# NLESC-JCER/Fortran_Davidson

Hardware: AMD Instinct MI355X
Metric: Davidson iterations/sec (dense DPR solve, matrix resident in HBM) + A*V HBM GB/s vs roofline (higher is better)
Workload: dtype f64

## Files before the change

### fortran_davidson_amd/csrc/engine_apply.hip

```cpp
#include "engine_internal.h"

bool inner_f32_tiles(E* e, OpDesc& o) {
  if (e->inner_bits != 32 || o.kind != DAV_KIND_DENSE || o.storage != 1 || o.a32_refused) return false;
  if (o.a32_valid) return true;
  const size_t count = (size_t)std::max<int64_t>(e->sym.ntiles, 1) * SYM_TB * SYM_TB;
  if (!o.a32 && pool_malloc(&o.a32, sizeof(float) * count) != hipSuccess) {
    (void)hipGetLastError();
    o.a32 = nullptr;
    o.a32_refused = true;
    return false;
  }
  launch_tiles_to_f32(e->stream, o.a, o.a32, (int64_t)count);
  o.a32_valid = true;
  return true;
}

static double* sym_slab_t(const E* e, const SymLaunch& L) { return e->sym_slab + (int64_t)L.ngroups * L.dstride; }
static void sym_sweep(E* e, const SymLaunch& L, const OpDesc& o, const SymSet& set, const double* xt) {
  if (L.nitems == 0) return;
  const SymPlan* pl = L.plan;
  const void* tiles = L.use32 ? (const void*)o.a32 : (const void*)o.a;
  double *slabD = e->sym_slab, *slabT = sym_slab_t(e, L);
  const int64_t xs = e->xt_group_stride, ds = L.dstride, ts = L.tstride;
  switch (L.family) {
    case SYM_ROW_STORED:
      return launch_matvec_sym(e->stream, o.a, set.row_off, set.items, set.nitems, xt, L.kk, slabD, slabT, L.ngroups, xs, ds, ts);
    case SYM_ROW_GENERATED:
      return launch_matvec_sym_generated(e->stream, op_params(o), e->n, set.items, set.nitems, xt, L.kk, slabD, slabT, L.ngroups, xs, ds, ts);
    case SYM_SUPER:
      return launch_matvec_sym9(e->stream, L.R, o.kind != DAV_KIND_DENSE, tiles, L.use32, set.row_off, o.kind != DAV_KIND_DENSE ? op_params(o) : OpParams{},
                                e->n, e->sym_nb, pl->items, pl->nitems, pl->zslot_begin, xt, L.kk, slabD, slabT, L.nwg, xs, ds, ts, e->tune.sym_mfma4 != 0);
    case SYM_WIDE:
    case SYM_WIDE_F32:
      return launch_matvec_symw(e->stream, L.nbw, L.tall, L.use32, tiles, set.row_off, e->sym_nb, pl->items, pl->nitems, pl->zslot_begin, xt, L.kk, slabD, slabT, L.nwg, xs, ds, ts);
    case SYM_WIDE_GENERATED:
      return launch_matvec_symw_generated(e->stream, op_params(o), e->n, e->sym_nb, pl->items, pl->nitems, pl->zslot_begin, xt, L.kk, slabD, slabT, L.nwg, xs, ds, ts);
  }
}

static void count_apply(E* e, int which, int kk) { if (which == DAV_OP_A) { e->st.applies += 1; e->st.apply_cols += kk; } }

static int pack_operand(E* e, const double* src, int kk, bool gather) {
  launch_pack_xt(e->stream, src, e->ldp, e->nloc, e->nslab, kk, e->xt, e->xt_group_stride, e->row0);
  if (!gather) return 0;
  const int ngroups = (kk + 15) / 16;
  CollGroup grp(e);
  CHK(grp.begin(5, 8.0 * (double)e->nslab * 16 * ngroups * e->nranks));
  for (int g = 0; g < ngroups; ++g)
    CHK(coll_allgather(e, e->xt + g * e->xt_group_stride + e->row0 * 16, e->xt + g * e->xt_group_stride, (size_t)e->nslab * 16));
  return grp.end("all-gather of the new block", e->stream);
}

static void sym_reduce_groups(E* e, const SymLaunch& L, const SymSet& set, const int64_t* owned, double* out, int64_t chunk_rows, bool accumulate) {
  const int64_t total_rows = (int64_t)e->nranks * e->nslab;
  const double* slabT = sym_slab_t(e, L);
  for (int g = 0; g < L.ngroups; ++g) {
    const int kg = std::min(16, L.kk - 16 * g);
    const double *d = e->sym_slab + g * L.dstride, *t = slabT + g * L.tstride;
    double* og = out + (size_t)g * 16 * (size_t)(chunk_rows ? total_rows : e->ldp);
    if (L.plan)
      launch_sym9_reduce(e->stream, d, t, L.plan->row_begin, L.plan->zslot_begin, owned, L.plan->next_owned, L.R, e->sym_nb, e->nloc, kg, og, e->ldp,
                         chunk_rows, total_rows, accumulate);
    else
      launch_sym_reduce(e->stream, d, t, set.row_begin, owned, e->sym_nb, e->nloc, kg, og, e->ldp, chunk_rows, total_rows, accumulate);
  }
}

static int ensure_sym_wpart(E* e) {
  if (e->sym_wpart) return 0;
  HIPCHK(pool_malloc(&e->sym_wpart, sizeof(double) * (size_t)e->nranks * (size_t)e->nslab * 64));
  HIPCHK(pool_malloc(&e->sym_wrecv, sizeof(double) * (size_t)e->nslab * 64));
  return 0;
}

static int sym_scatter_to_panel(E* e, int kk, double* dst, bool accumulate, const char* what, double* h0 = nullptr, size_t h0_count = 0) {
  const size_t wstride = (size_t)e->nranks * (size_t)e->nslab * 16, rstride = (size_t)e->nslab * 16;
  const int ngroups = (kk + 15) / 16;
  CollGroup grp(e);
  CHK(grp.begin(6, 8.0 * (double)e->nslab * kk * e->nranks));
  for (int g = 0; g < ngroups; ++g)
    CHK(coll_reduce_scatter(e, e->sym_wpart + g * wstride, e->sym_wrecv + g * rstride, (size_t)e->nslab * std::min(16, kk - 16 * g)));
  if (h0) CHK(coll_allreduce(e, h0, h0_count));
  CHK(grp.end(what, e->stream));
  for (int g = 0; g < ngroups; ++g)
    launch_chunk_to_panel(e->stream, e->sym_wrecv + g * rstride, e->nslab, e->nloc, e->nloc_pad, std::min(16, kk - 16 * g), dst + (int64_t)(16 * g) * e->ldp, e->ldp, accumulate);
  return 0;
}

static double sym_stored_bytes(const E* e, const OpDesc& o, const SymSet& set, bool partial, bool use32) {
  return o.kind != DAV_KIND_DENSE ? 0.0 : (use32 ? 4.0 : 8.0) * (partial ? (double)set.ntiles * SYM_TB * SYM_TB : 0.5 * (double)e->n * ((double)e->n + 1.0) / e->nranks);
}

static int apply_sym_overlapped(E* e, int which, OpDesc& o, const double* src, int k, double* dst, bool timed, bool inner) {
  const int step = 32;
  const int nchunks = (k + step - 1) / step;
// ... 535 lines not shown
```

### fortran_davidson_amd/csrc/engine_comm.hip

```cpp
#include "engine_internal.h"

Rccl g_rccl;
int rccl_load() {
  if (g_rccl.lib) return 0;
  void* lib = dlopen("librccl.so", RTLD_NOW | RTLD_LOCAL);
  if (!lib) lib = dlopen("/opt/rocm/lib/librccl.so", RTLD_NOW | RTLD_LOCAL);
  if (!lib) return fail(std::string("cannot load librccl.so: ") + dlerror());
#define SYM(field, name)                                              \
  *(void**)(&g_rccl.field) = dlsym(lib, name);                        \
  if (!g_rccl.field) return fail(std::string("librccl.so lacks ") + name);
  SYM(GetUniqueId, "ncclGetUniqueId")
  SYM(CommInitRank, "ncclCommInitRank")
  SYM(CommDestroy, "ncclCommDestroy")
  SYM(AllGather, "ncclAllGather")
  SYM(AllReduce, "ncclAllReduce")
  SYM(Broadcast, "ncclBroadcast")
  SYM(ReduceScatter, "ncclReduceScatter")
  SYM(Send, "ncclSend")
  SYM(Recv, "ncclRecv")
  SYM(GroupStart, "ncclGroupStart")
  SYM(GroupEnd, "ncclGroupEnd")
  SYM(GetErrorString, "ncclGetErrorString")
  SYM(CommCount, "ncclCommCount")
#undef SYM
// ... 99 lines not shown
};
static void lg_release_turn(LocalGroup* g, int rank) {
  if (!g->serialize || g->segment[rank] == 0) return;
  const uint64_t pos = (uint64_t)((rank - g->first + g->n) % g->n);
  { std::lock_guard<std::mutex> lk(g->mu); g->turn = std::max(g->turn, g->segment[rank] * (uint64_t)g->n + pos + 1); }
  g->cv.notify_all();
}
static void lg_acquire_turn(LocalGroup* g, int rank) {
  if (!g->serialize) return;
  g->segment[rank] += 1;
  const uint64_t pos = (uint64_t)((rank - g->first + g->n) % g->n);
  const uint64_t ticket = g->segment[rank] * (uint64_t)g->n + pos;
  std::unique_lock<std::mutex> lk(g->mu);
  if (pos == 0 && g->turn < ticket) g->turn = ticket;
  g->cv.notify_all();
  g->cv.wait(lk, [&] { return g->turn >= ticket; });
}

struct ShmHeader {
  pthread_barrier_t bar;
  int nranks;
  size_t slot_doubles;
};
struct ShmGroup {
  ShmHeader* hdr = nullptr;
  double* slots = nullptr;
  size_t bytes = 0;
  std::string name;
  bool owner = false;
};

bool has_test_transport(const E* e) { return e->lg != nullptr || e->shm != nullptr; }
size_t test_transport_max_message(const E* e) { return e->shm ? e->shm->hdr->slot_doubles : (size_t)-1; }

int test_allgather(E* e, const double* send, double* recv, size_t count) {
  if (e->lg) {
    LocalGroup* g = e->lg;
    HIPCHK(hipStreamSynchronize(e->stream));
    lg_release_turn(g, e->rank);
    g->send[e->rank] = send;
    pthread_barrier_wait(&g->bar);
    for (int p = 0; p < g->n; ++p)
      if (recv + (size_t)p * count != g->send[p])
        HIPCHK(hipMemcpyAsync(recv + (size_t)p * count, g->send[p], sizeof(double) * count, hipMemcpyDeviceToDevice, e->stream));
    HIPCHK(hipStreamSynchronize(e->stream));
    pthread_barrier_wait(&g->bar);
    lg_acquire_turn(g, e->rank);
    return 0;
  }
  if (e->shm) {
    ShmGroup* g = e->shm;
    if (count > g->hdr->slot_doubles) return fail("shared-memory transport: message larger than a slot");
    HIPCHK(hipMemcpyAsync(g->slots + (size_t)e->rank * g->hdr->slot_doubles, send, sizeof(double) * count, hipMemcpyDeviceToHost, e->stream));
    HIPCHK(hipStreamSynchronize(e->stream));
    pthread_barrier_wait(&g->hdr->bar);
    for (int p = 0; p < e->nranks; ++p)
      if (p != e->rank || recv + (size_t)p * count != send)
        HIPCHK(hipMemcpyAsync(recv + (size_t)p * count, g->slots + (size_t)p * g->hdr->slot_doubles, sizeof(double) * count,
                              hipMemcpyHostToDevice, e->stream));
    HIPCHK(hipStreamSynchronize(e->stream));
    pthread_barrier_wait(&g->hdr->bar);
    return 0;
  }
  return fail("no test transport");
}

// ... 124 lines not shown
    for (int tries = 0; tries < 3000 && __atomic_load_n(&g->hdr->nranks, __ATOMIC_ACQUIRE) != e->nranks; ++tries) usleep(10000);
    if (__atomic_load_n(&g->hdr->nranks, __ATOMIC_ACQUIRE) != e->nranks) { munmap(p, bytes); delete g; return fail("dav_comm_init_shm: rank 0 did not initialise the segment"); }
  }
  e->shm = g;
  pthread_barrier_wait(&g->hdr->bar);
  return 0;
}

extern "C" int dav_local_group_yield(dav_handle_t e) {
  if (!e || !e->lg) return 0;
  (void)hipSetDevice(e->device);
  (void)hipStreamSynchronize(e->stream);
  lg_release_turn(e->lg, e->rank);
  return 0;
}

extern "C" int dav_local_group_join(dav_handle_t* handles, int n) {
  if (!handles || n < 1 || n > 16) return fail("dav_local_group_join: 1..16 engines");
  for (int r = 0; r < n; ++r)
    if (!handles[r] || handles[r]->nranks != n || handles[r]->rank != r || handles[r]->lg || handles[r]->comm)
      return fail("dav_local_group_join: engine r must be created with rank r of n and have no transport yet");
  LocalGroup* g = new LocalGroup();
  g->n = n;
  if (const char* ev = getenv("DAV_TEST_SERIALIZE")) g->serialize = ev[0] == '1';
  if (const char* ev = getenv("DAV_TEST_SERIALIZE_FIRST")) g->first = std::max(0, std::min(n - 1, atoi(ev)));
  pthread_barrier_init(&g->bar, nullptr, (unsigned)n);
  for (int r = 0; r < n; ++r) handles[r]->lg = g;
  return 0;
}

#else
bool has_test_transport(const E*) { return false; }
size_t test_transport_max_message(const E*) { return (size_t)-1; }
int test_allgather(E*, const double*, double*, size_t) { return fail("built without test transports"); }
int test_allreduce(E*, double*, size_t) { return fail("built without test transports"); }
int test_reduce_scatter(E*, const double*, double*, size_t) { return fail("built without test transports"); }
void shm_release(E*) {}
#endif

#if DAV_TEST_TRANSPORTS
__global__ void watchdog_stall_kernel(unsigned long long ticks) {
  const unsigned long long t0 = __builtin_amdgcn_s_memrealtime();
  while (__builtin_amdgcn_s_memrealtime() - t0 < ticks) __builtin_amdgcn_s_sleep(64);
}
#endif
int watch_mark(E* e, const char* what, hipStream_t stream) {
  Watchdog* w = e->wd;
  if (!w || e->group_depth > 0) return 0;
#if DAV_TEST_TRANSPORTS
  static const long stall_ms = [] { const char* ev = getenv("DAV_TEST_STALL_MS"); return ev ? atol(ev) : 0L; }();
  static const long stall_from = [] { const char* ev = getenv("DAV_TEST_STALL_FROM"); return ev ? atol(ev) : 0L; }();
  if (stall_ms > 0 && (long)w->seq >= stall_from)
    hipLaunchKernelGGL(watchdog_stall_kernel, dim3(1), dim3(1), 0, stream, (unsigned long long)stall_ms * 100000ull);
#endif
  std::lock_guard<std::mutex> lk(w->mu);
  Watchdog::Lane* l = nullptr;
  for (Watchdog::Lane& c : w->lane)
    if (c.used && c.stream == stream) { l = &c; break; }
  if (!l)
    for (Watchdog::Lane& c : w->lane)
      if (!c.used) { c.used = true; c.stream = stream; l = &c; break; }
  if (!l) return fail("collective watchdog: more streams than lanes");
  Watchdog::Mark& m = l->check_active ? l->latest : l->check;
  HIPCHK(hipEventRecord(m.ev, stream));
  m.what = what; m.seq = w->seq++; m.t0 = wall_seconds(); m.iter = e->iter_hint;
  if (l->check_active) l->latest_valid = true;
// ... 144 lines not shown
```

### fortran_davidson_amd/csrc/engine_internal.h

```cpp
#pragma once
#include "davidson_hip_private.h"
#include "kernels.h"
#include "ingest.h"

#include <dlfcn.h>
#include <fcntl.h>
#include <pthread.h>
#include <sys/mman.h>
#include <sys/stat.h>
#include <unistd.h>
#include <rccl/rccl.h>

#include <algorithm>
#include <chrono>
#include <condition_variable>
#include <ctime>
#include <mutex>
#include <cmath>
#include <cstdio>
#include <cstring>
#include <numeric>
#include <string>
#include <thread>
#include <vector>
// ... 130 lines not shown
  int64_t res_tiles = 0;
  int res_first = 0;
  bool res_decided = false;
  bool pass_res = false, pass_gen = false;
  SymSet* res = nullptr;
  SymSet* gen = nullptr;
  dav_device_apply_fn dev_fn = nullptr;
  void* dev_ctx = nullptr;
  SparseStore sp;
};

struct SmallBuf {
  double* dev = nullptr;
  double* host = nullptr;
  hipEvent_t done = nullptr;
  bool pending = false;
};

constexpr int N_SMALL = 4;
constexpr int N_EVPAIRS = 64;

struct Tune {
  int sym_wide = 2;
  int sym_wide32 = 1;
  int sym_pair = 1;
  int sym_quad = 1;
  int sym_overlap = 0;
  int sym_r = 0;
  int sym_tall = 1;
  int sym_gen_wide = 1;
  int sym_run = 0;
  int sym_run9 = 0;
  int sym_mfma4 = 1;
  int64_t mv_target = 0;
  int64_t mv_nsplit = 0;
  int gram_wgs = 0;
  int pg_pin = 1;
  int coll_direct = 0;
  int b_resident = 1;
  bool gjd_trace = false;
  int coll_select = 1;
  int coll_trial_corrupt = 0;
  bool coll_forced = false;
  int no_h0 = 0;
  int harness_libm = 0;
  int cheb_fuse = 1;
};
Tune tune_from_env();

enum { COLL_PATH_UNDECIDED = -1, COLL_PATH_PROGRAM_ORDER = 0, COLL_PATH_DIRECT = 1, COLL_PATH_SECOND_STREAM = 2 };
struct CollTrial {
  bool ran = false;
  int selected = COLL_PATH_PROGRAM_ORDER, columns = 0;
  double ms[3] = {0, 0, 0}, ms_max[3] = {0, 0, 0};
  bool valid[3] = {true, false, false}, valid_all[3] = {true, false, false};
  double differing[3] = {0, 0, 0}, maxdiff[3] = {0, 0, 0};
  std::string message[3];
};

enum { GUESS_NONE = 0, GUESS_ONE_SHOT = 1, GUESS_RESULT = 2 };
struct Watchdog;
struct dav_engine {
  Tune tune;
  int device = 0;
  hipStream_t stream = nullptr;
  int64_t n = 0, nslab = 0, nloc = 0, row0 = 0, nloc_pad = 0, ncols_pad = 0;
// ... 99 lines not shown
  bool stop = false;
  uint64_t seq = 0;
  double timeout_s = 0.0;
  int device = 0, rank = 0, nranks = 1;
};

static inline int method_kind(int code) { return code > 0 && (code & 0xff) == DAV_METHOD_CHEB ? DAV_METHOD_CHEB : code; }
static inline int64_t roundup(int64_t x, int64_t m) { return (x + m - 1) / m * m; }

struct SmallMat {
  const double* src; int64_t ld; int p, q;
  double* dev; int64_t ldm;
  bool image = false;
};

int bind(E* e);
int collect_events(E* e);
int timed_begin(E* e, int kind, double bytes, int* slot);
int timed_end(E* e, int slot);
int timed_begin_on(E* e, int kind, double bytes, int* slot, hipStream_t stream);
int timed_end_on(E* e, int slot, hipStream_t stream);
int small_upload(E* e, int i, const double* src, int64_t ld, int p, int q, int64_t* ldm_out);
int small_upload_multi(E* e, int i, SmallMat* mats, int n);
int small_upload_image(E* e, int i, const double* src, int64_t ld, int p, int q, int64_t* tp_out);
double* panel_ptr(E* e, int panel, int col);
int check_panel(E* e, int panel, int c0, int k);
int create_impl(E* e, int device, int64_t n, int max_cols, int gev, int rank, int nranks);
double wall_seconds();
void watchdog_loop(Watchdog* w);
bool has_comm(E* e);
int need_comm(E* e);
bool has_test_transport(const E* e);
size_t test_transport_max_message(const E* e);
int test_allgather(E* e, const double* send, double* recv, size_t count);
int test_allreduce(E* e, double* buf, size_t count);
int test_reduce_scatter(E* e, const double* send, double* recv, size_t count);
void shm_release(E* e);
int watch_mark(E* e, const char* what, hipStream_t stream);
int coll_group_begin(E* e);
int coll_group_end(E* e, const char* what, hipStream_t stream);
void coll_group_abort(E* e);
struct CollGroup {
  E* e; bool open = false; int slot = -1;
  explicit CollGroup(E* e_) : e(e_) {}
  int begin(int kind = 0, double bytes = 0.0, hipStream_t stream = nullptr) {
    if (kind != 0) {
      int rc = timed_begin_on(e, kind, bytes, &slot, stream ? stream : e->stream);
      if (rc != 0) return rc;
      e->st.collectives += 1;
      e->group_timed = true;
    }
    int rc = coll_group_begin(e); open = rc == 0; return rc;
  }
  int end(const char* what, hipStream_t stream) {
    open = false;
    e->group_timed = false;
    int rc = coll_group_end(e, what, stream);
    if (rc != 0) return rc;
    return timed_end_on(e, slot, stream);
  }
  ~CollGroup() { e->group_timed = false; if (open) coll_group_abort(e); }
};
int coll_allgather(E* e, const double* send, double* recv, size_t count);
int coll_allreduce(E* e, double* buf, size_t count);
int coll_reduce_scatter(E* e, const double* send, double* recv, size_t count);
int refresh_diag_host(E* e, int which);
// ... 42 lines not shown
```

### fortran_davidson_amd/csrc/k_matvec_sym9.hip

```cpp
#include "kernels.h"
#include <cstdlib>
#include <type_traits>

__device__ __forceinline__ const double* sym9_tile(const double* tiles, const int64_t* __restrict__ row_off, int I, int J) {
  return tiles + (row_off[I] + J) * (int64_t)(SYM_TB * SYM_TB);
}

__device__ __forceinline__ double mfma4_f64(double a, double b, double c) { return __builtin_amdgcn_mfma_f64_4x4x4f64(a, b, c, 0, 0, 0); }

template <int R, bool GEN, bool F32, bool M4, int HARN = 0>
__global__ __launch_bounds__(512, 1) void matvec_sym9_kernel(const void* __restrict__ tiles_v, const int64_t* __restrict__ row_off,
                                                             const int* __restrict__ items,
                                                             const int* __restrict__ zslot_begin, const double* __restrict__ xt,
                                                             double* __restrict__ slabD, double* __restrict__ slabT, int kcols,
                                                             int npair, int64_t xt_gstride, int64_t slabD_gstride,
                                                             int64_t slabT_gstride, int nb, OpParams op, int64_t n) {
  const double* tiles = static_cast<const double*>(tiles_v);
  const float* tiles32 = static_cast<const float*>(tiles_v);
  (void)tiles; (void)tiles32;
  constexpr int NCG = 4 / R;
  constexpr int NRS = 2 * R;
  constexpr int BW = 16 * NCG;
  constexpr int UPJ = SYM_TB / BW;
  constexpr int UPS = 64 / BW;
// ... 324 lines not shown
                     kcols, npair, xt_gstride, slabD_gstride, slabT_gstride, nb, op, n)
  const bool harness = gen && op.kind == DAV_KIND_HARNESS;
  const bool hsin = harness && op.trig != 0;
  const bool hlibm = harness && op.libm != 0;
  if (R == 4) {
    if (hlibm) DAV_SYM9_LAUNCH(4, true, false, true, 3);
    else if (hsin) DAV_SYM9_LAUNCH(4, true, false, true, 2);
    else if (harness) DAV_SYM9_LAUNCH(4, true, false, true, 1);
    else if (gen) DAV_SYM9_LAUNCH(4, true, false, true);
    else if (tiles_f32) DAV_SYM9_LAUNCH(4, false, true, true);
    else if (m4) DAV_SYM9_LAUNCH(4, false, false, true);
    else DAV_SYM9_LAUNCH(4, false, false, false);
  } else {
    if (hlibm) DAV_SYM9_LAUNCH(2, true, false, false, 3);
    else if (hsin) DAV_SYM9_LAUNCH(2, true, false, false, 2);
    else if (harness) DAV_SYM9_LAUNCH(2, true, false, false, 1);
    else if (gen) DAV_SYM9_LAUNCH(2, true, false, false);
    else if (tiles_f32) DAV_SYM9_LAUNCH(2, false, true, false);
    else DAV_SYM9_LAUNCH(2, false, false, false);
  }
#undef DAV_SYM9_LAUNCH
}

__global__ __launch_bounds__(256) void tiles_to_f32_kernel(const double* __restrict__ src, float* __restrict__ dst, int64_t count4) {
  for (int64_t e = (int64_t)blockIdx.x * 256 + threadIdx.x; e < count4; e += (int64_t)gridDim.x * 256) {
    const f64x2 a = reinterpret_cast<const f64x2*>(src)[2 * e], b = reinterpret_cast<const f64x2*>(src)[2 * e + 1];
    reinterpret_cast<float4*>(dst)[e] = float4{(float)a.x, (float)a.y, (float)b.x, (float)b.y};
  }
}
void launch_tiles_to_f32(hipStream_t st, const double* src, float* dst, int64_t count) {
  hipLaunchKernelGGL(tiles_to_f32_kernel, dim3(256 * 32), dim3(256), 0, st, src, dst, count / 4);
}

__global__ __launch_bounds__(256) void sym9_reduce_kernel(const double* __restrict__ slabD, const double* __restrict__ slabT,
                                                          const int* __restrict__ row_item_begin, const int* __restrict__ zslot_begin,
                                                          const int64_t* __restrict__ owned, const int* __restrict__ next_owned, int R, int nb,
                                                          int nsuper, int64_t nloc, int k, double* __restrict__ dst, int64_t ldd,
                                                          int64_t chunk_rows, int64_t total_rows, int accumulate) {
  const int J = blockIdx.x, col = blockIdx.y, r = threadIdx.x;
  if (col >= k) return;
  double sum = 0.0;
  const int Sown = J / R, sub = J % R;
  for (int it = row_item_begin[Sown]; it < row_item_begin[Sown + 1]; ++it)
    sum += slabD[(((int64_t)it * R + sub) * 16 + col) * SYM_TB + r];
  auto zt = [&](int S) { return slabT[(((int64_t)zslot_begin[S] + J) * 16 + col) * SYM_TB + r]; };
  double s0 = 0.0, s1 = 0.0, s2 = 0.0, s3 = 0.0;
  const int Send = (nb - 1 > J) ? nsuper : 0;
  if (!owned) {
    int S = (J + 1) / R;
    for (; S + 3 < Send; S += 4) { s0 += zt(S); s1 += zt(S + 1); s2 += zt(S + 2); s3 += zt(S + 3); }
    for (; S < Send; ++S) s0 += zt(S);
  } else {
    int S = (J + 1) / R < nsuper ? next_owned[(J + 1) / R] : nsuper;
    while (S < Send) {
      s0 += zt(S); S = next_owned[S + 1];
      if (S >= Send) break;
      s1 += zt(S); S = next_owned[S + 1];
      if (S >= Send) break;
      s2 += zt(S); S = next_owned[S + 1];
      if (S >= Send) break;
      s3 += zt(S); S = next_owned[S + 1];
    }
  }
  sum += (s0 + s1) + (s2 + s3);
  const int64_t row = (int64_t)J * SYM_TB + r;
  if (chunk_rows > 0) {
    if (row < total_rows) dst[(row / chunk_rows) * (chunk_rows * k) + (int64_t)col * chunk_rows + row % chunk_rows] = sum;
  } else {
    dst[(int64_t)col * ldd + row] = row < nloc ? (accumulate ? dst[(int64_t)col * ldd + row] + sum : sum) : 0.0;
  }
}

void launch_sym9_reduce(hipStream_t st, const double* slabD, const double* slabT, const int* row_item_begin_dev,
                        const int* zslot_begin_dev, const int64_t* owned, const int* next_owned, int R, int nb, int64_t nloc, int k, double* dst,
                        int64_t ldd, int64_t chunk_rows, int64_t total_rows, bool accumulate) {
  const int nsuper = (nb + R - 1) / R;
  hipLaunchKernelGGL(sym9_reduce_kernel, dim3(nb, k), dim3(256), 0, st, slabD, slabT, row_item_begin_dev, zslot_begin_dev, owned, next_owned, R,
                     nb, nsuper, nloc, k, dst, ldd, chunk_rows, total_rows, accumulate && chunk_rows == 0 ? 1 : 0);
}
```

### fortran_davidson_amd/csrc/kernels.h

```cpp
#pragma once
#include "common.h"

constexpr int MV_ROWS = 256;
void launch_pack_xt(hipStream_t st, const double* src, int64_t ld, int64_t nloc, int64_t nslab, int k,
                    double* xt, int64_t xt_group_stride, int64_t row_off);
void launch_matvec_dense(hipStream_t st, const double* A, int64_t lda, int64_t nrows_pad, int64_t ncols_pad,
                         const double* xt, int64_t xt_group_stride, int ngroups, double* slab,
                         int nsplit, int jc);
void launch_matvec_free(hipStream_t st, OpParams op, int64_t row0, int64_t nloc, int64_t n,
                        int64_t nrows_pad, int64_t ncols_pad, const double* xt, int64_t xt_group_stride,
                        int ngroups, double* slab, int nsplit, int jc);
void launch_slab_reduce(hipStream_t st, const double* slab, int nsplit, int64_t nrows_pad, int ngroups,
                        int64_t nloc, int k, double* dst, int64_t ldd);
size_t matvec_slab_doubles(int64_t nrows_pad, int ngroups, int nsplit);
void matvec_plan(int64_t nrows_pad, int64_t ncols_pad, int ngroups, int* nsplit, int* jc, int64_t target = 0, int64_t forced_nsplit = 0);

constexpr int GRAM_MIN_ROWS = 256;
constexpr int GRAM_FUSE_CHUNKS = 24;
constexpr int GRAM_MAX_COUNTERS = 256;
void launch_gram(hipStream_t st, const double* P, int64_t ldp, int p, const double* Q, int64_t ldq, int q,
                 int64_t nrows_pad, double* scratch, double* out_dev, unsigned* counters = nullptr, int wg_target = 0);
size_t gram_scratch_doubles(int p, int q, int64_t nrows_pad);
void gram_set_fuse_chunks(int n);
void launch_gram_multi(hipStream_t st, const double* P, int64_t ldp, int p, const double* const* Qs, int nq, int qeach, int64_t ldq,
// ... 44 lines not shown

struct LincombArgs {
  const double* in[4]; const double* coef; int ldc; int nterms;
  double* out; int64_t ld; int64_t nrows_pad; int m;
};
void launch_lincomb(hipStream_t st, const LincombArgs& a);
void launch_precond(hipStream_t st, const double* in, double* out, int64_t ld, int64_t nloc, int64_t nrows_pad, int m,
                    const double* theta, const double* dA, const double* dB, const double* active);
struct DotsArgs {
  const double* a[4]; const double* b[4]; int npairs; int64_t ld; int64_t nrows_pad; int m; double* partial;
};
int coldots_blocks(int64_t nrows_pad);
void launch_coldots(hipStream_t st, const DotsArgs& a);

constexpr int SYM_TB = 256;
void launch_matvec_sym(hipStream_t st, const double* tiles, const int64_t* row_off, const int* items_dev, int nitems, const double* xt, int kcols,
                       double* slabD, double* slabT, int npair, int64_t xt_gstride, int64_t slabD_gstride, int64_t slabT_gstride);
void launch_matvec_sym_generated(hipStream_t st, OpParams op, int64_t n, const int* items_dev, int nitems, const double* xt, int kcols,
                                 double* slabD, double* slabT, int npair, int64_t xt_gstride, int64_t slabD_gstride,
                                 int64_t slabT_gstride);
void launch_sym_reduce(hipStream_t st, const double* slabD, const double* slabT, const int* row_item_begin_dev, const int64_t* owned,
                       int nb, int64_t nloc, int k, double* dst, int64_t ldd, int64_t chunk_rows, int64_t total_rows, bool accumulate = false);
void launch_matvec_sym9(hipStream_t st, int R, bool gen, const void* tiles, bool tiles_f32, const int64_t* row_off, OpParams op, int64_t n,
                        int nb, const int* items_dev, int nitems, const int* zslot_begin_dev, const double* xt, int kcols, double* slabD,
                        double* slabT, int npair, int64_t xt_gstride, int64_t slabD_gstride, int64_t slabT_gstride, bool mfma4 = true);
void launch_matvec_symw(hipStream_t st, int nbw, bool tall, bool tiles_f32, const void* tiles, const int64_t* row_off, int nb, const int* items_dev,
                        int nitems, const int* zslot_begin_dev, const double* xt, int kcols, double* slabD, double* slabT, int nwg,
                        int64_t xt_gstride, int64_t slabD_gstride, int64_t slabT_gstride);
void launch_matvec_symw_generated(hipStream_t st, OpParams op, int64_t n, int nb, const int* items_dev, int nitems, const int* zslot_begin_dev,
                                  const double* xt, int kcols, double* slabD, double* slabT, int nwg, int64_t xt_gstride, int64_t slabD_gstride,
                                  int64_t slabT_gstride);
void launch_tiles_to_f32(hipStream_t st, const double* src, float* dst, int64_t count);
void launch_sym9_reduce(hipStream_t st, const double* slabD, const double* slabT, const int* row_item_begin_dev,
                        const int* zslot_begin_dev, const int64_t* owned, const int* next_owned, int R, int nb, int64_t nloc, int k, double* dst,
                        int64_t ldd, int64_t chunk_rows, int64_t total_rows, bool accumulate = false);
void launch_generate_sym_tiles(hipStream_t st, double* tiles, const int64_t* row_off_host, int nb, int64_t n, uint64_t seed,
                               double sparsity, int use_diag, double diag_val);
void launch_retile_panel(hipStream_t st, const double* panel, int64_t ldp, int64_t nrows, int ncols, int J, int nb,
                         const int64_t* row_off, double* tiles);
void launch_diag_sym(hipStream_t st, const double* tiles, const int64_t* row_off, int64_t n, int64_t nrows, double* diag);
void launch_gather_columns_sym_rs(hipStream_t st, const double* tiles, const int64_t* row_off, int64_t n, int64_t chunk_rows,
                                  int64_t total_rows, const int64_t* idx_dev, int k, double* dst);
void launch_entries_sym(hipStream_t st, const double* tiles, const int64_t* row_off, const int64_t* idx_dev, int k, double* h0);
void launch_zero_pad_rows(hipStream_t st, double* dst, int64_t ldd, int64_t nloc, int64_t nrows_pad, int k);
void launch_entries_free(hipStream_t st, OpParams op, const int64_t* idx_dev, int k, double* h0);
void launch_entries_dense(hipStream_t st, const double* A, int64_t lda, const int64_t* idx_dev, int k, double* h0);
void launch_gather_columns_free(hipStream_t st, OpParams op, int64_t row0, int64_t nloc, int64_t nrows_pad, const int64_t* idx_dev, int k,
                                double* dst, int64_t ldd);
void launch_gather_columns_sym(hipStream_t st, const double* tiles, const int64_t* row_off, int64_t n, int64_t nrows_pad,
                               const int64_t* idx_dev, int k, double* dst, int64_t ldd);
void launch_chunk_to_panel(hipStream_t st, const double* src, int64_t lds, int64_t nloc, int64_t nrows_pad, int k, double* dst, int64_t ldd,
                           bool accumulate = false);

constexpr int CSR_ROWS = 16;
constexpr int64_t CSR_CHUNK = 1024;
struct CsrItem { int64_t p0, p1; int32_t row, nrows, slot, pad; };
struct CsrLong { int32_t row, first, count, pad; };
void launch_spmm_csr(hipStream_t st, const CsrItem* items, int nitems, const int64_t* rp, const int32_t* col, const double* val,
                     const double* xt, int64_t xt_gstride, int groups, int kk, double* part, double* dst, int64_t ldd);
void launch_spmm_csr_finish(hipStream_t st, const CsrLong* longs, int nlong, const double* part, int kk, double* dst, int64_t ldd);
struct ChebEpi { const double *z, *r, *zprev, *hdr, *ab, *pi; int64_t ld; };
void launch_spmm_csr_cheb(hipStream_t st, const CsrItem* items, int nitems, const int64_t* rp, const int32_t* col, const double* val,
                          const double* xt, int64_t xt_gstride, int groups, int kk, double* part, double* dst, int64_t ldd, const ChebEpi& epi);
void launch_spmm_csr_finish_cheb(hipStream_t st, const CsrLong* longs, int nlong, const double* part, int kk, double* dst, int64_t ldd,
                                 const ChebEpi& epi);

template <class F> void cb_dispatch(int rp64, int ci64, F&& f) {
  if (rp64) {
// ... 93 lines not shown
```

### fortran_davidson_amd/csrc/engine.hip

```cpp
#include "engine_internal.h"

thread_local std::string g_err;
int fail(const std::string& msg) {
  g_err = msg;
  return 1;
}

int bind(E* e) {
  e->h0_take = e->h0_cols;
  e->h0_cols = 0;
  HIPCHK(hipSetDevice(e->device));
  return 0;
}

int collect_events(E* e) {
  e->ev_open = 0;
  for (int i = 0; i < e->ev_used; ++i) {
    if (!e->ev_done[i]) continue;
    HIPCHK(hipEventSynchronize(e->ev[i][1]));
    float ms = 0;
    HIPCHK(hipEventElapsedTime(&ms, e->ev[i][0], e->ev[i][1]));
    if (e->ev_kind[i] == 0) {
      e->st.apply_ms += ms;
      e->st.apply_bytes += e->ev_bytes[i];
// ... 129 lines not shown
extern "C" int dav_create(dav_handle_t* h, int device, int64_t n, int max_cols, int gev, int rank, int nranks) {
  if (!h || n <= 0 || max_cols <= 0 || nranks <= 0 || rank < 0 || rank >= nranks) return fail("dav_create: bad arguments");
  *h = nullptr;
  int ndev = 0;
  HIPCHK(hipGetDeviceCount(&ndev));
  if (ndev <= 0) return fail("dav_create: no HIP device visible - the HIP path has no CPU fallback");
  if (device < 0 || device >= ndev) return fail("dav_create: device index out of range");
  E* e = new E();
  int rc = create_impl(e, device, n, max_cols, gev, rank, nranks);
  if (rc != 0) {
    std::string msg = g_err;
    dav_destroy(e);
    g_err = msg;
    return rc;
  }
  *h = e;
  return 0;
}

Tune tune_from_env() {
  Tune t;
  auto geti = [](const char* name, int dflt) { const char* ev = getenv(name); return ev && *ev ? atoi(ev) : dflt; };
  t.sym_wide = geti("DAV_SYM_WIDE", t.sym_wide);
  t.sym_wide32 = geti("DAV_SYM_WIDE32", t.sym_wide32);
  t.sym_pair = geti("DAV_SYM_PAIR", t.sym_pair);
  t.sym_quad = geti("DAV_SYM_QUAD", t.sym_quad);
  t.sym_overlap = geti("DAV_SYM_OVERLAP", t.sym_overlap);
  t.sym_r = geti("DAV_SYM_R", t.sym_r);
  t.sym_tall = geti("DAV_SYM_TALL", t.sym_tall);
  t.sym_gen_wide = geti("DAV_SYM_GEN_WIDE", 1);
  t.sym_run = std::max(0, geti("DAV_SYM_RUN", 0));
  t.sym_run9 = std::max(0, geti("DAV_SYM_RUN9", 0));
  t.sym_mfma4 = geti("DAV_SYM_MFMA4", t.sym_mfma4);
  t.mv_target = std::max(0, geti("DAV_MV_TARGET", 0));
  t.mv_nsplit = std::max(0, geti("DAV_MV_NSPLIT", 0));
  t.b_resident = geti("DAV_B_RESIDENT", t.b_resident);
  t.coll_direct = geti("DAV_COLL_DIRECT", t.coll_direct);
  t.pg_pin = geti("DAV_PG_PIN", t.pg_pin);
  t.gram_wgs = geti("DAV_GRAM_WGS", t.gram_wgs);
  gram_set_fuse_chunks(geti("DAV_GRAM_FUSE", 0));
  t.gjd_trace = getenv("DAV_GJD_TRACE") != nullptr;
  t.harness_libm = geti("DAV_HARNESS_LIBM", 0);
  t.no_h0 = geti("DAV_NO_H0", 0);
  t.cheb_fuse = geti("DAV_CHEB_FUSE", t.cheb_fuse);
  t.coll_select = geti("DAV_COLL_SELECT", 1);
  t.coll_trial_corrupt = geti("DAV_COLL_TRIAL_CORRUPT", 0);
  t.coll_forced = getenv("DAV_SYM_OVERLAP") != nullptr || getenv("DAV_COLL_DIRECT") != nullptr;
  return t;
}

namespace {
struct PoolBlock { void* p; size_t bytes; int device; int kind; uint64_t gen; };
struct Pool {
  std::mutex mu;
  std::vector<PoolBlock> live, idle;
  std::vector<std::pair<int, hipStream_t>> streams;
  uint64_t gen = 0;
  int enabled = -1;
  size_t cap_bytes = 0;
  size_t cap_pinned_bytes = 0;
  int destroying = 0;
};
Pool& pool() { static Pool* p = new Pool; return *p; }
constexpr size_t POOL_MIN_BYTES = 64 << 10;

bool pool_enabled(Pool& P) {
// ... 439 lines not shown
```

Measured before the change: 23.73.

## Replace per-group symmetric reduce launches with single streaming reduce kernel

Replaces the per-16-column-group loop of sym reduce launches with one kernel whose grid covers tile rows and column groups. Each 1024-thread block sums the transposed-slot and diagonal-slab contributions using nontemporal vector loads, with four independent accumulators software-pipelined across sched barriers to keep several loads in flight. The aim is to cut launch overhead and raise the memory-level parallelism of this bandwidth-bound reduction. The old per-group path is kept behind an environment variable, at the cost of a fair amount of new specialised code (four ownership modes, full and partial column groups).

Result: no change. 23.79 (median of 2 runs) (+0.2%).

```diff
diff --git a/fortran_davidson_amd/csrc/engine_apply.hip b/fortran_davidson_amd/csrc/engine_apply.hip
--- a/fortran_davidson_amd/csrc/engine_apply.hip
+++ b/fortran_davidson_amd/csrc/engine_apply.hip
@@ -54,6 +54,17 @@
 static void sym_reduce_groups(E* e, const SymLaunch& L, const SymSet& set, const int64_t* owned, double* out, int64_t chunk_rows, bool accumulate) {
   const int64_t total_rows = (int64_t)e->nranks * e->nslab;
   const double* slabT = sym_slab_t(e, L);
+  if (!test_reduce_per_group()) {
+    SymReduceStream a;
+    a.slabD = e->sym_slab; a.slabT = slabT; a.dstride = L.dstride; a.tstride = L.tstride;
+    a.row_item_begin = L.plan ? L.plan->row_begin : set.row_begin;
+    a.zslot_begin = L.plan ? L.plan->zslot_begin : nullptr;
+    a.owned = owned; a.next_owned = L.plan ? L.plan->next_owned : nullptr;
+    a.R = L.plan ? L.R : 1; a.nb = e->sym_nb; a.nsuper = (a.nb + a.R - 1) / a.R; a.kk = L.kk;
+    a.nloc = e->nloc; a.dst = out; a.ldd = e->ldp; a.chunk_rows = chunk_rows; a.total_rows = total_rows;
+    a.accumulate = accumulate && chunk_rows == 0 ? 1 : 0;
+    return launch_sym_reduce_stream(e->stream, a);
+  }
   for (int g = 0; g < L.ngroups; ++g) {
     const int kg = std::min(16, L.kk - 16 * g);
     const double *d = e->sym_slab + g * L.dstride, *t = slabT + g * L.tstride;
diff --git a/fortran_davidson_amd/csrc/engine_comm.hip b/fortran_davidson_amd/csrc/engine_comm.hip
--- a/fortran_davidson_amd/csrc/engine_comm.hip
+++ b/fortran_davidson_amd/csrc/engine_comm.hip
@@ -155,6 +155,7 @@
 
 bool has_test_transport(const E* e) { return e->lg != nullptr || e->shm != nullptr; }
 size_t test_transport_max_message(const E* e) { return e->shm ? e->shm->hdr->slot_doubles : (size_t)-1; }
+bool test_reduce_per_group() { const char* ev = getenv("DAV_TEST_REDUCE_PER_GROUP"); return ev && ev[0] == '1'; }
 
 int test_allgather(E* e, const double* send, double* recv, size_t count) {
   if (e->lg) {
@@ -345,6 +346,7 @@
 #else
 bool has_test_transport(const E*) { return false; }
 size_t test_transport_max_message(const E*) { return (size_t)-1; }
+bool test_reduce_per_group() { return false; }
 int test_allgather(E*, const double*, double*, size_t) { return fail("built without test transports"); }
 int test_allreduce(E*, double*, size_t) { return fail("built without test transports"); }
 int test_reduce_scatter(E*, const double*, double*, size_t) { return fail("built without test transports"); }
diff --git a/fortran_davidson_amd/csrc/engine_internal.h b/fortran_davidson_amd/csrc/engine_internal.h
--- a/fortran_davidson_amd/csrc/engine_internal.h
+++ b/fortran_davidson_amd/csrc/engine_internal.h
@@ -351,6 +351,7 @@
 int need_comm(E* e);
 bool has_test_transport(const E* e);
 size_t test_transport_max_message(const E* e);
+bool test_reduce_per_group();
 int test_allgather(E* e, const double* send, double* recv, size_t count);
 int test_allreduce(E* e, double* buf, size_t count);
 int test_reduce_scatter(E* e, const double* send, double* recv, size_t count);
diff --git a/fortran_davidson_amd/csrc/k_matvec_sym9.hip b/fortran_davidson_amd/csrc/k_matvec_sym9.hip
--- a/fortran_davidson_amd/csrc/k_matvec_sym9.hip
+++ b/fortran_davidson_amd/csrc/k_matvec_sym9.hip
@@ -426,3 +426,163 @@
   hipLaunchKernelGGL(sym9_reduce_kernel, dim3(nb, k), dim3(256), 0, st, slabD, slabT, row_item_begin_dev, zslot_begin_dev, owned, next_owned, R,
                      nb, nsuper, nloc, k, dst, ldd, chunk_rows, total_rows, accumulate && chunk_rows == 0 ? 1 : 0);
 }
+
+constexpr int SRS_NT = 1024, SRS_U = 2;
+constexpr int SRS_CP = SRS_NT / 128;
+template <bool FULL>
+__device__ __forceinline__ void srs_load(f64x2 (&x)[SRS_U], const double* __restrict__ slot, int t, int nu) {
+#pragma unroll
+  for (int u = 0; u < SRS_U; ++u)
+    x[u] = __builtin_nontemporal_load(reinterpret_cast<const f64x2*>(slot) + (FULL || u < nu ? u : 0) * SRS_NT + t);
+}
+__device__ __forceinline__ void srs_add(f64x2 (&s)[SRS_U], const f64x2 (&x)[SRS_U]) {
+#pragma unroll
+  for (int u = 0; u < SRS_U; ++u) s[u] = s[u] + x[u];
+}
+
+template <bool FULL, int MODE>
+__device__ __forceinline__ void sym_reduce_stream_body(const SymReduceStream& a, const int* __restrict__ row_item_begin,
+                                                       const int* __restrict__ zslot_begin, const int64_t* __restrict__ owned,
+                                                       const int* __restrict__ next_owned, const int J, const int g, const int kg, const int t) {
+  constexpr int64_t SLOT = 16 * SYM_TB;
+  const int part = t >> 7;
+  const int nu = FULL ? SRS_U : __builtin_amdgcn_readfirstlane((kg + SRS_CP - 1 - part) / SRS_CP);
+  const double* __restrict__ slabD = a.slabD + g * a.dstride;
+  const double* __restrict__ slabT = a.slabT + g * a.tstride;
+  auto tslot = [&](int S) {
+    const int64_t z = (MODE == 0 || MODE == 1) ? (int64_t)zslot_begin[S] : (int64_t)S * (S - 1) / 2;
+    return slabT + (z + J) * SLOT;
+  };
+  f64x2 s0[SRS_U], s1[SRS_U], s2[SRS_U], s3[SRS_U], x0[SRS_U], x1[SRS_U], x2[SRS_U], x3[SRS_U];
+#pragma unroll
+  for (int u = 0; u < SRS_U; ++u) s0[u] = s1[u] = s2[u] = s3[u] = f64x2{0.0, 0.0};
+  const int Sfirst = (J + 1) / a.R;
+  const int Send = (a.nb - 1 > J) ? a.nsuper : 0;
+  if (MODE == 0 || MODE == 3) {
+    const int n = Send - Sfirst;
+    int q = 0;
+    if (n >= 8) {
+      srs_load<FULL>(x0, tslot(Sfirst), t, nu);
+      __builtin_amdgcn_sched_barrier(0);
+      srs_load<FULL>(x1, tslot(Sfirst + 1), t, nu);
+      __builtin_amdgcn_sched_barrier(0);
+      srs_load<FULL>(x2, tslot(Sfirst + 2), t, nu);
+      __builtin_amdgcn_sched_barrier(0);
+      srs_load<FULL>(x3, tslot(Sfirst + 3), t, nu);
+      __builtin_amdgcn_sched_barrier(0);
+    } else {
+      if (0 < n) srs_load<FULL>(x0, tslot(Sfirst), t, nu);
+      if (1 < n) srs_load<FULL>(x1, tslot(Sfirst + 1), t, nu);
+      if (2 < n) srs_load<FULL>(x2, tslot(Sfirst + 2), t, nu);
+      if (3 < n) srs_load<FULL>(x3, tslot(Sfirst + 3), t, nu);
+    }
+    for (; q + 7 < n; q += 4) {
+      srs_add(s0, x0);
+      srs_load<FULL>(x0, tslot(Sfirst + q + 4), t, nu);
+      __builtin_amdgcn_sched_barrier(0);
+      srs_add(s1, x1);
+      srs_load<FULL>(x1, tslot(Sfirst + q + 5), t, nu);
+      __builtin_amdgcn_sched_barrier(0);
+      srs_add(s2, x2);
+      srs_load<FULL>(x2, tslot(Sfirst + q + 6), t, nu);
+      __builtin_amdgcn_sched_barrier(0);
+      srs_add(s3, x3);
+      srs_load<FULL>(x3, tslot(Sfirst + q + 7), t, nu);
+      __builtin_amdgcn_sched_barrier(0);
+    }
+    if (q + 3 < n) {
+      srs_add(s0, x0);
+      if (q + 4 < n) srs_load<FULL>(x0, tslot(Sfirst + q + 4), t, nu);
+      srs_add(s1, x1);
+      if (q + 5 < n) srs_load<FULL>(x1, tslot(Sfirst + q + 5), t, nu);
+      srs_add(s2, x2);
+      if (q + 6 < n) srs_load<FULL>(x2, tslot(Sfirst + q + 6), t, nu);
+      srs_add(s3, x3);
+      q += 4;
+    }
+    if (q < n) srs_add(s0, x0);
+    if (q + 1 < n) srs_add(s0, x1);
+    if (q + 2 < n) srs_add(s0, x2);
+  } else if (MODE == 1) {
+    int S = Sfirst < a.nsuper ? next_owned[Sfirst] : a.nsuper;
+    while (S < Send) {
+      const int Sa = S;
+      const int Sb = next_owned[Sa + 1];
+      const int Sc = Sb < Send ? next_owned[Sb + 1] : Send;
+      const int Sd = Sc < Send ? next_owned[Sc + 1] : Send;
+      srs_load<FULL>(x0, tslot(Sa), t, nu);
+      if (Sb < Send) srs_load<FULL>(x1, tslot(Sb), t, nu);
+      if (Sc < Send) srs_load<FULL>(x2, tslot(Sc), t, nu);
+      if (Sd < Send) srs_load<FULL>(x3, tslot(Sd), t, nu);
+      srs_add(s0, x0);
+      if (Sb < Send) srs_add(s1, x1);
+      if (Sc < Send) srs_add(s2, x2);
+      if (Sd < Send) srs_add(s3, x3);
+      S = Sd < Send ? next_owned[Sd + 1] : Send;
+    }
+  } else {
+    auto own = [&](int I) { return owned[I] >= 0; };
+    int I = Sfirst;
+    for (; I + 3 < Send; I += 4) {
+      const bool o0 = own(I), o1 = own(I + 1), o2 = own(I + 2), o3 = own(I + 3);
+      if (o0) srs_load<FULL>(x0, tslot(I), t, nu);
+      if (o1) srs_load<FULL>(x1, tslot(I + 1), t, nu);
+      if (o2) srs_load<FULL>(x2, tslot(I + 2), t, nu);
+      if (o3) srs_load<FULL>(x3, tslot(I + 3), t, nu);
+      if (o0) srs_add(s0, x0);
+      if (o1) srs_add(s1, x1);
+      if (o2) srs_add(s2, x2);
+      if (o3) srs_add(s3, x3);
+    }
+    for (; I < Send; ++I)
+      if (own(I)) { srs_load<FULL>(x0, tslot(I), t, nu); srs_add(s0, x0); }
+  }
+#pragma unroll
+  for (int u = 0; u < SRS_U; ++u) s0[u] = (s0[u] + s1[u]) + (s2[u] + s3[u]);
+#pragma unroll
+  for (int u = 0; u < SRS_U; ++u) s1[u] = f64x2{0.0, 0.0};
+  const int Sown = J / a.R, sub = J % a.R;
+  const int it1 = row_item_begin[Sown + 1];
+  for (int it = row_item_begin[Sown]; it < it1; it += 2) {
+    srs_load<FULL>(x0, slabD + ((int64_t)it * a.R + sub) * SLOT, t, nu);
+    if (it + 1 < it1) srs_load<FULL>(x1, slabD + ((int64_t)(it + 1) * a.R + sub) * SLOT, t, nu);
+    srs_add(s1, x0);
+    if (it + 1 < it1) srs_add(s1, x1);
+  }
+  const int r0 = 2 * (t & 127);
+  double* __restrict__ dst = a.dst + (int64_t)g * 16 * (a.chunk_rows > 0 ? a.total_rows : a.ldd);
+#pragma unroll
+  for (int u = 0; u < SRS_U; ++u) {
+    if (!(FULL || u < nu)) continue;
+    const f64x2 v = s1[u] + s0[u];
+    const int col = SRS_CP * u + part;
+#pragma unroll
+    for (int h = 0; h < 2; ++h) {
+      const int64_t row = (int64_t)J * SYM_TB + r0 + h;
+      if (a.chunk_rows > 0) {
+        if (row < a.total_rows) dst[(row / a.chunk_rows) * (a.chunk_rows * kg) + (int64_t)col * a.chunk_rows + row % a.chunk_rows] = v[h];
+      } else {
+        double* p = dst + (int64_t)col * a.ldd + row;
+        *p = row < a.nloc ? (a.accumulate ? *p + v[h] : v[h]) : 0.0;
+      }
+    }
+  }
+}
+
+template <int MODE>
+__global__ __launch_bounds__(SRS_NT) void sym_reduce_stream_kernel(const SymReduceStream a, const int* __restrict__ row_item_begin,
+                                                                   const int* __restrict__ zslot_begin, const int64_t* __restrict__ owned,
+                                                                   const int* __restrict__ next_owned) {
+  const int J = blockIdx.x, g = blockIdx.y;
+  const int kg = min(16, a.kk - 16 * g);
+  if (kg == 16) sym_reduce_stream_body<true, MODE>(a, row_item_begin, zslot_begin, owned, next_owned, J, g, kg, threadIdx.x);
+  else sym_reduce_stream_body<false, MODE>(a, row_item_begin, zslot_begin, owned, next_owned, J, g, kg, threadIdx.x);
+}
+
+void launch_sym_reduce_stream(hipStream_t st, const SymReduceStream& a) {
+  const dim3 grid(a.nb, (a.kk + 15) / 16), block(SRS_NT);
+  if (!a.owned && a.zslot_begin) hipLaunchKernelGGL(sym_reduce_stream_kernel<0>, grid, block, 0, st, a, a.row_item_begin, a.zslot_begin, a.owned, a.next_owned);
+  else if (!a.owned) hipLaunchKernelGGL(sym_reduce_stream_kernel<3>, grid, block, 0, st, a, a.row_item_begin, a.zslot_begin, a.owned, a.next_owned);
+  else if (a.next_owned) hipLaunchKernelGGL(sym_reduce_stream_kernel<1>, grid, block, 0, st, a, a.row_item_begin, a.zslot_begin, a.owned, a.next_owned);
+  else hipLaunchKernelGGL(sym_reduce_stream_kernel<2>, grid, block, 0, st, a, a.row_item_begin, a.zslot_begin, a.owned, a.next_owned);
+}
diff --git a/fortran_davidson_amd/csrc/kernels.h b/fortran_davidson_amd/csrc/kernels.h
--- a/fortran_davidson_amd/csrc/kernels.h
+++ b/fortran_davidson_amd/csrc/kernels.h
@@ -102,6 +102,13 @@
 void launch_sym9_reduce(hipStream_t st, const double* slabD, const double* slabT, const int* row_item_begin_dev,
                         const int* zslot_begin_dev, const int64_t* owned, const int* next_owned, int R, int nb, int64_t nloc, int k, double* dst,
                         int64_t ldd, int64_t chunk_rows, int64_t total_rows, bool accumulate = false);
+struct SymReduceStream {
+  const double* slabD; const double* slabT; int64_t dstride, tstride;
+  const int* row_item_begin; const int* zslot_begin; const int64_t* owned; const int* next_owned;
+  int R, nb, nsuper, kk;
+  int64_t nloc; double* dst; int64_t ldd, chunk_rows, total_rows; int accumulate;
+};
+void launch_sym_reduce_stream(hipStream_t st, const SymReduceStream& a);
 void launch_generate_sym_tiles(hipStream_t st, double* tiles, const int64_t* row_off_host, int nb, int64_t n, uint64_t seed,
                                double sparsity, int use_diag, double diag_val);
 void launch_retile_panel(hipStream_t st, const double* panel, int64_t ldp, int64_t nrows, int ncols, int J, int nb,
```

## Replace per-group sym9 reduce with single fused multi-group vectorized reduce kernel

Applied to the files above, without the earlier changes.

Adds a new sym9 reduce kernel that handles all 16-column groups in one launch, with column slices of 8 per block, f64x2 non-temporal loads and 4-way unrolled independent accumulators over diagonal items and transposed slots. It replaces the old per-group launches of the reference kernel, which stays available behind DAV_SYM_REDUCE=0. The aim is to cut launch overhead and raise memory-level parallelism in the reduction of the symmetric matvec slabs. The different summation order changes floating-point rounding slightly.

New measurement: 24.07 before, 24.16 after, median of 6. No clear change (+0.4%).

```diff
diff --git a/fortran_davidson_amd/csrc/engine.hip b/fortran_davidson_amd/csrc/engine.hip
--- a/fortran_davidson_amd/csrc/engine.hip
+++ b/fortran_davidson_amd/csrc/engine.hip
@@ -185,6 +185,7 @@
   t.sym_run = std::max(0, geti("DAV_SYM_RUN", 0));
   t.sym_run9 = std::max(0, geti("DAV_SYM_RUN9", 0));
   t.sym_mfma4 = geti("DAV_SYM_MFMA4", t.sym_mfma4);
+  t.sym_reduce = geti("DAV_SYM_REDUCE", t.sym_reduce);
   t.mv_target = std::max(0, geti("DAV_MV_TARGET", 0));
   t.mv_nsplit = std::max(0, geti("DAV_MV_NSPLIT", 0));
   t.b_resident = geti("DAV_B_RESIDENT", t.b_resident);
diff --git a/fortran_davidson_amd/csrc/engine_apply.hip b/fortran_davidson_amd/csrc/engine_apply.hip
--- a/fortran_davidson_amd/csrc/engine_apply.hip
+++ b/fortran_davidson_amd/csrc/engine_apply.hip
@@ -54,13 +54,17 @@
 static void sym_reduce_groups(E* e, const SymLaunch& L, const SymSet& set, const int64_t* owned, double* out, int64_t chunk_rows, bool accumulate) {
   const int64_t total_rows = (int64_t)e->nranks * e->nslab;
   const double* slabT = sym_slab_t(e, L);
+  const int64_t ostride = 16 * (chunk_rows ? total_rows : e->ldp);
+  if (L.plan && e->tune.sym_reduce != 0)
+    return launch_sym9_reduce(e->stream, e->sym_slab, slabT, L.plan->row_begin, L.plan->zslot_begin, owned, L.plan->next_owned, L.R, e->sym_nb, e->nloc,
+                              L.kk, L.dstride, L.tstride, out, e->ldp, ostride, chunk_rows, total_rows, accumulate);
   for (int g = 0; g < L.ngroups; ++g) {
     const int kg = std::min(16, L.kk - 16 * g);
     const double *d = e->sym_slab + g * L.dstride, *t = slabT + g * L.tstride;
-    double* og = out + (size_t)g * 16 * (size_t)(chunk_rows ? total_rows : e->ldp);
+    double* og = out + g * ostride;
     if (L.plan)
-      launch_sym9_reduce(e->stream, d, t, L.plan->row_begin, L.plan->zslot_begin, owned, L.plan->next_owned, L.R, e->sym_nb, e->nloc, kg, og, e->ldp,
-                         chunk_rows, total_rows, accumulate);
+      launch_sym9_reduce_ref(e->stream, d, t, L.plan->row_begin, L.plan->zslot_begin, owned, L.plan->next_owned, L.R, e->sym_nb, e->nloc, kg, og, e->ldp,
+                             chunk_rows, total_rows, accumulate);
     else
       launch_sym_reduce(e->stream, d, t, set.row_begin, owned, e->sym_nb, e->nloc, kg, og, e->ldp, chunk_rows, total_rows, accumulate);
   }
diff --git a/fortran_davidson_amd/csrc/engine_internal.h b/fortran_davidson_amd/csrc/engine_internal.h
--- a/fortran_davidson_amd/csrc/engine_internal.h
+++ b/fortran_davidson_amd/csrc/engine_internal.h
@@ -186,6 +186,7 @@
   int sym_run = 0;
   int sym_run9 = 0;
   int sym_mfma4 = 1;
+  int sym_reduce = 1;
   int64_t mv_target = 0;
   int64_t mv_nsplit = 0;
   int gram_wgs = 0;
diff --git a/fortran_davidson_amd/csrc/k_matvec_sym9.hip b/fortran_davidson_amd/csrc/k_matvec_sym9.hip
--- a/fortran_davidson_amd/csrc/k_matvec_sym9.hip
+++ b/fortran_davidson_amd/csrc/k_matvec_sym9.hip
@@ -380,7 +380,7 @@
   hipLaunchKernelGGL(tiles_to_f32_kernel, dim3(256 * 32), dim3(256), 0, st, src, dst, count / 4);
 }
 
-__global__ __launch_bounds__(256) void sym9_reduce_kernel(const double* __restrict__ slabD, const double* __restrict__ slabT,
+__global__ __launch_bounds__(256) void sym9_reduce_ref_kernel(const double* __restrict__ slabD, const double* __restrict__ slabT,
                                                           const int* __restrict__ row_item_begin, const int* __restrict__ zslot_begin,
                                                           const int64_t* __restrict__ owned, const int* __restrict__ next_owned, int R, int nb,
                                                           int nsuper, int64_t nloc, int k, double* __restrict__ dst, int64_t ldd,
@@ -419,10 +419,142 @@
   }
 }
 
-void launch_sym9_reduce(hipStream_t st, const double* slabD, const double* slabT, const int* row_item_begin_dev,
+void launch_sym9_reduce_ref(hipStream_t st, const double* slabD, const double* slabT, const int* row_item_begin_dev,
                         const int* zslot_begin_dev, const int64_t* owned, const int* next_owned, int R, int nb, int64_t nloc, int k, double* dst,
                         int64_t ldd, int64_t chunk_rows, int64_t total_rows, bool accumulate) {
   const int nsuper = (nb + R - 1) / R;
-  hipLaunchKernelGGL(sym9_reduce_kernel, dim3(nb, k), dim3(256), 0, st, slabD, slabT, row_item_begin_dev, zslot_begin_dev, owned, next_owned, R,
+  hipLaunchKernelGGL(sym9_reduce_ref_kernel, dim3(nb, k), dim3(256), 0, st, slabD, slabT, row_item_begin_dev, zslot_begin_dev, owned, next_owned, R,
                      nb, nsuper, nloc, k, dst, ldd, chunk_rows, total_rows, accumulate && chunk_rows == 0 ? 1 : 0);
 }
+
+constexpr int SYM9_RED_CW = 8;
+template <int NC, bool FULL>
+__device__ __forceinline__ void sym9_reduce_sums(const double* __restrict__ dp, int64_t ditem, int it0, int it1, const double* __restrict__ tp,
+                                                 const int* __restrict__ zslot_begin, const int64_t* __restrict__ owned,
+                                                 const int* __restrict__ next_owned, int S0, int Send, int nsuper, int nc, f64x2 (&sum)[NC]) {
+  constexpr int64_t CSTEP = 2 * SYM_TB;
+  auto ld = [&](const double* p, int i) {
+    return (FULL || i < nc) ? __builtin_nontemporal_load(reinterpret_cast<const f64x2*>(p + i * CSTEP)) : f64x2{0.0, 0.0};
+  };
+  int it = it0;
+  for (; it + 3 < it1; it += 4) {
+    f64x2 v[4][NC];
+#pragma unroll
+    for (int u = 0; u < 4; ++u)
+#pragma unroll
+      for (int i = 0; i < NC; ++i) v[u][i] = ld(dp + (it + u) * ditem, i);
+#pragma unroll
+    for (int u = 0; u < 4; ++u)
+#pragma unroll
+      for (int i = 0; i < NC; ++i) sum[i] += v[u][i];
+  }
+  for (; it < it1; ++it)
+#pragma unroll
+    for (int i = 0; i < NC; ++i) sum[i] += ld(dp + it * ditem, i);
+  f64x2 s[4][NC];
+#pragma unroll
+  for (int u = 0; u < 4; ++u)
+#pragma unroll
+    for (int i = 0; i < NC; ++i) s[u][i] = f64x2{0.0, 0.0};
+  auto zp = [&](int S) { return tp + (int64_t)zslot_begin[S] * (16 * SYM_TB); };
+  if (!owned) {
+    int S = S0;
+    for (; S + 3 < Send; S += 4) {
+      f64x2 v[4][NC];
+#pragma unroll
+      for (int u = 0; u < 4; ++u) {
+        const double* p = zp(S + u);
+#pragma unroll
+        for (int i = 0; i < NC; ++i) v[u][i] = ld(p, i);
+      }
+#pragma unroll
+      for (int u = 0; u < 4; ++u)
+#pragma unroll
+        for (int i = 0; i < NC; ++i) s[u][i] += v[u][i];
+    }
+    for (; S < Send; ++S) {
+      const double* p = zp(S);
+#pragma unroll
+      for (int i = 0; i < NC; ++i) s[0][i] += ld(p, i);
+    }
+  } else {
+    int S = S0 < nsuper ? next_owned[S0] : nsuper;
+    while (S < Send) {
+      const double* p[4];
+      int cnt = 0;
+#pragma unroll
+      for (int u = 0; u < 4; ++u) {
+        p[u] = tp;
+        if (S < Send) { p[u] = zp(S); S = next_owned[S + 1]; cnt = u + 1; }
+      }
+      f64x2 v[4][NC];
+#pragma unroll
+      for (int u = 0; u < 4; ++u)
+#pragma unroll
+        for (int i = 0; i < NC; ++i) v[u][i] = u < cnt ? ld(p[u], i) : f64x2{0.0, 0.0};
+#pragma unroll
+      for (int u = 0; u < 4; ++u)
+        if (u < cnt) {
+#pragma unroll
+          for (int i = 0; i < NC; ++i) s[u][i] += v[u][i];
+        }
+    }
+  }
+#pragma unroll
+  for (int i = 0; i < NC; ++i) sum[i] += (s[0][i] + s[1][i]) + (s[2][i] + s[3][i]);
+}
+
+__global__ __launch_bounds__(256) void sym9_reduce_kernel(const double* __restrict__ slabD, const double* __restrict__ slabT,
+                                                          const int* __restrict__ row_item_begin, const int* __restrict__ zslot_begin,
+                                                          const int64_t* __restrict__ owned, const int* __restrict__ next_owned, int R, int nb,
+                                                          int nsuper, int64_t nloc, int k, int64_t dstride, int64_t tstride,
+                                                          double* __restrict__ dst, int64_t ldd, int64_t ostride, int64_t chunk_rows,
+                                                          int64_t total_rows, int accumulate) {
+  constexpr int CW = SYM9_RED_CW, NSL = 16 / CW, NC = CW / 2;
+  const int nper = (k + CW - 1) / CW;
+  const int J = blockIdx.x / nper, rem = blockIdx.x % nper, g = rem / NSL, c0 = (rem % NSL) * CW;
+  const int kg = min(16, k - 16 * g);
+  const int ch = threadIdx.x >> 7, rp = threadIdx.x & 127;
+  const int ncol = min(CW, kg - c0), nc = ncol > ch ? (ncol - ch + 1) / 2 : 0;
+  const int Sown = J / R, sub = J % R;
+  const int64_t toff = (int64_t)(c0 + ch) * SYM_TB + 2 * rp;
+  const double* dp = slabD + g * dstride + (int64_t)sub * (16 * SYM_TB) + toff;
+  const double* tp = slabT + g * tstride + (int64_t)J * (16 * SYM_TB) + toff;
+  const int Send = (nb - 1 > J) ? nsuper : 0;
+  f64x2 sum[NC];
+#pragma unroll
+  for (int i = 0; i < NC; ++i) sum[i] = f64x2{0.0, 0.0};
+  if (nc == NC)
+    sym9_reduce_sums<NC, true>(dp, (int64_t)R * 16 * SYM_TB, row_item_begin[Sown], row_item_begin[Sown + 1], tp, zslot_begin, owned, next_owned,
+                               (J + 1) / R, Send, nsuper, nc, sum);
+  else
+    sym9_reduce_sums<NC, false>(dp, (int64_t)R * 16 * SYM_TB, row_item_begin[Sown], row_item_begin[Sown + 1], tp, zslot_begin, owned, next_owned,
+                                (J + 1) / R, Send, nsuper, nc, sum);
+  const int64_t row = (int64_t)J * SYM_TB + 2 * rp;
+  double* og = dst + g * ostride;
+#pragma unroll
+  for (int i = 0; i < NC; ++i) {
+    if (i >= nc) break;
+    const int col = c0 + ch + 2 * i;
+    if (chunk_rows > 0) {
+      if (row < total_rows) *reinterpret_cast<f64x2*>(og + (row / chunk_rows) * (chunk_rows * kg) + (int64_t)col * chunk_rows + row % chunk_rows) = sum[i];
+    } else {
+      f64x2* o = reinterpret_cast<f64x2*>(og + (int64_t)col * ldd + row);
+      f64x2 v = sum[i];
+      if (accumulate) { const f64x2 old = *o; v = old + v; }
+      if (row >= nloc) v.x = 0.0;
+      if (row + 1 >= nloc) v.y = 0.0;
+      *o = v;
+    }
+  }
+}
+
+void launch_sym9_reduce(hipStream_t st, const double* slabD, const double* slabT, const int* row_item_begin_dev,
+                        const int* zslot_begin_dev, const int64_t* owned, const int* next_owned, int R, int nb, int64_t nloc, int k,
+                        int64_t dstride, int64_t tstride, double* dst, int64_t ldd, int64_t ostride, int64_t chunk_rows, int64_t total_rows,
+                        bool accumulate) {
+  const int nsuper = (nb + R - 1) / R;
+  hipLaunchKernelGGL(sym9_reduce_kernel, dim3((unsigned)nb * ((k + SYM9_RED_CW - 1) / SYM9_RED_CW)), dim3(256), 0, st, slabD, slabT,
+                     row_item_begin_dev, zslot_begin_dev, owned, next_owned, R, nb, nsuper, nloc, k, dstride, tstride, dst, ldd, ostride,
+                     chunk_rows, total_rows, accumulate && chunk_rows == 0 ? 1 : 0);
+}
diff --git a/fortran_davidson_amd/csrc/kernels.h b/fortran_davidson_amd/csrc/kernels.h
--- a/fortran_davidson_amd/csrc/kernels.h
+++ b/fortran_davidson_amd/csrc/kernels.h
@@ -100,8 +100,12 @@
                                   int64_t slabT_gstride);
 void launch_tiles_to_f32(hipStream_t st, const double* src, float* dst, int64_t count);
 void launch_sym9_reduce(hipStream_t st, const double* slabD, const double* slabT, const int* row_item_begin_dev,
-                        const int* zslot_begin_dev, const int64_t* owned, const int* next_owned, int R, int nb, int64_t nloc, int k, double* dst,
-                        int64_t ldd, int64_t chunk_rows, int64_t total_rows, bool accumulate = false);
+                        const int* zslot_begin_dev, const int64_t* owned, const int* next_owned, int R, int nb, int64_t nloc, int k,
+                        int64_t dstride, int64_t tstride, double* dst, int64_t ldd, int64_t ostride, int64_t chunk_rows, int64_t total_rows,
+                        bool accumulate);
+void launch_sym9_reduce_ref(hipStream_t st, const double* slabD, const double* slabT, const int* row_item_begin_dev,
+                            const int* zslot_begin_dev, const int64_t* owned, const int* next_owned, int R, int nb, int64_t nloc, int k, double* dst,
+                            int64_t ldd, int64_t chunk_rows, int64_t total_rows, bool accumulate = false);
 void launch_generate_sym_tiles(hipStream_t st, double* tiles, const int64_t* row_off_host, int nb, int64_t n, uint64_t seed,
                                double sparsity, int use_diag, double diag_val);
 void launch_retile_panel(hipStream_t st, const double* panel, int64_t ldp, int64_t nrows, int ncols, int J, int nb,
```
